# segeschecho/OpenEKFMonoSLAM

Measured on AMD Instinct MI355X. Metric: EKF updates/s (frames/s) at N features, higher is better.
Workload: dtype f32 storage; i8 MFMA with exact i32 sums (downdate) + f64 (B, S, state)

## Files before the change

### openekfmonoslam_amd/csrc/engine.cpp

```cpp
#include "engine.h"
#include "../../include/ekf_test_hooks.h"

#include <cmath>
#include <cstdio>
#include <algorithm>
#include <atomic>
#include <cstdlib>
#include <chrono>
#include <cstring>
#include <mutex>
#include <new>

#include <dlfcn.h>
#include <rccl/rccl.h>

using namespace ekf;

namespace ekf {
void launch_partition(EkfEngine *e, const EkfMatch *src, int M, const uint8_t *flags, EkfMatch *dst1, EkfMatch *dst0,
                      int *cnt1, bool map_update = false, const uint8_t *d_kdesc = nullptr, int *d_idx0 = nullptr,
                      int publish_seq = 0, bool rescue = false);
void launch_outlier_idx(EkfEngine *e, const EkfMatch *src, int M, int *idx);
}

// ... 1374 lines not shown
        }
        (void)hipEventDestroy(e->sw_events[i].first);
        (void)hipEventDestroy(e->sw_events[i].second);
    }
    e->sw_events.clear();
    e->sw_launch.clear();
    e->sw_m.clear();
}

struct StageTimer {
    EkfEngine *e;
    std::vector<hipEvent_t> evs;
    explicit StageTimer(EkfEngine *eng) : e(eng) {}
    ~StageTimer()
    {
        for (auto ev : evs) (void)hipEventDestroy(ev);
    }
    void mark()
    {
        if (!e->timing) return;
        hipEvent_t ev;
        if (hipEventCreate(&ev) != hipSuccess) return;
        (void)hipEventRecord(ev, e->stream);
        evs.push_back(ev);
    }
    void finish()
    {
        if (!e->timing || evs.size() < 7) return;
        (void)hipStreamSynchronize(e->stream);
        double *dst[6] = {&e->times.prediction_ms, &e->times.matching_ms, &e->times.ransac_ms,
                          &e->times.update_li_ms,  &e->times.rescue_ms,   &e->times.update_hi_ms};
        for (int i = 0; i < 6; ++i) {
            float ms = 0.f;
            if (hipEventElapsedTime(&ms, evs[i], evs[i + 1]) == hipSuccess) *dst[i] += ms;
        }
        for (auto ev : evs) (void)hipEventDestroy(ev);
        evs.clear();
        e->times.steps += 1;
        harvest_pu_events(e);
    }
};

static int match_ncc_dev(EkfEngine *e, int *n_matches);

static int detect_step_keypoints(EkfEngine *e);

static int step_dev(EkfEngine *e, const EkfKeypoint *d_kps, const uint8_t *d_desc, int n_kp, EkfStepInfo *info,
                    bool use_ncc = false, bool detect = false)
{
    const bool dev_counts = !use_ncc && !detect && !e->img.valid && !e->keep_step_preds && e->shard_world == 1;
    const bool lean = e->shard_world > 1;
    int *cnt = e->d.counts;
    EkfStepInfo li;
    std::memset(&li, 0, sizeof(li));
    int status = EKF_OK, rc;
    const int retries0 = e->sweep_retries;
    if (!dev_counts && e->err_unread) {
        if ((rc = read_counts(e))) return rc;
        if ((rc = recover_failed_update(e, &status))) return rc;
    }
    bool restarted = false;
restart:
    StageTimer tm(e);
    tm.mark();
    int np = 0;
    if (dev_counts) {
        const bool deferred = launch_predict_with_features(e, e->N);
        launch_hp_rows(e, e->d.plist, e->N, true, cnt + CNT_NPRED, deferred);
    } else {
        launch_predict(e);
        if ((rc = predict_measurements_dev(e, nullptr, e->N, &np, true, lean))) return rc;
    }
    tm.mark();
    int M = 0;
    if (dev_counts) {
        launch_match(e, d_kps, d_desc, e->N, n_kp, cnt + CNT_NPRED, true);
    } else {
        if (detect && (rc = detect_step_keypoints(e))) return rc;
        if (lean) rc = match_sharded_dev(e, use_ncc, d_kps, d_desc, n_kp, &M);
        else rc = use_ncc ? match_ncc_dev(e, &M) : match_dev(e, d_kps, d_desc, n_kp, &M, detect ? cnt + CNT_KP_FOUND : nullptr);
        if (rc) return rc;
    }
    tm.mark();
    if (dev_counts) {
        const int batch = e->cfg.ransac_batch;
        const int seq_r = next_publish_seq(e);
        launch_ransac_batch(e, e->N, 0, batch, cnt + CNT_NMATCH, seq_r);
        if ((rc = wait_counts(e, seq_r))) return rc;
        if (e->h_counts[CNT_ERR] && !restarted) {
            if ((rc = recover_failed_update(e, &status))) return rc;
            restarted = true;
            goto restart;
        }
        np = e->n_pred = e->h_counts[CNT_NPRED];
        M = e->h_counts[CNT_NMATCH];
        for (int h0 = batch, nb = batch * RANSAC_WIDE_FACTOR; !e->h_counts[CNT_RS_DONE] && h0 < M; h0 += nb) {
            launch_ransac_batch(e, M, h0, nb);
            if ((rc = read_counts(e))) return rc;
        }
    } else if (M > 0 && (rc = ransac_dev(e, M, lean))) {
        return rc;
    }
    li.n_predicted = np;
    li.n_matches = M;
    int ni = 0, no = 0;
    if (M > 0) {
        li.n_hypotheses = e->h_counts[CNT_RS_NEXT];
        ni = e->h_counts[CNT_RS_BEST];
        no = M - ni;
        launch_partition(e, e->d.matches, M, e->d.best_flags, e->d.msel, e->d.mout, nullptr, true, d_desc, e->d.work_idx);
    }
    li.n_inliers = ni;
    li.n_outliers = no;
    tm.mark();
    if ((rc = update_dev(e, ni, true, lean))) return rc;
    tm.mark();
    int nr = 0;
    if (no > 0) {
        int nop = 0;
        for (int attempt = 0; attempt < 2; ++attempt) {
            if (dev_counts) {
                launch_predict_features(e, e->d.work_idx, no, false);
                launch_hp_rows(e, e->d.plist_sub, no, false, cnt + CNT_NPRED_SUB);
                const int seq_p = next_publish_seq(e);
                launch_partition(e, e->d.mout, no, e->d.mask, e->d.msel, nullptr, cnt + CNT_NRESC, true, d_desc, nullptr, seq_p, true);
                rc = wait_counts(e, seq_p);
            } else {
                rc = predict_measurements_dev(e, e->d.work_idx, no, &nop, false, lean);
            }
            if (rc) return rc;
            if (!e->h_counts[CNT_ERR]) break;
            if ((rc = recover_failed_update(e, &status))) return rc;
        }
        if (dev_counts) {
            nr = e->h_counts[CNT_NRESC];
        } else if (nop > 0) {
            launch_rescue(e, e->d.mout, no);
            launch_partition(e, e->d.mout, no, e->d.mask, e->d.msel, nullptr, cnt + CNT_NRESC, true, d_desc);
            if ((rc = read_counts(e))) return rc;
            nr = e->h_counts[CNT_NRESC];
        }
    }
    li.n_rescued = nr;
    tm.mark();
    if ((rc = update_dev(e, nr, true, lean))) return rc;
    tm.mark();
    if (dev_counts && e->async_errors) {
        e->err_unread = true;
    } else {
        if ((rc = read_counts(e))) return rc;
        if (detect) {
            e->step_kp_detected = e->h_counts[CNT_KP_FOUND];
            e->step_kp_kept = std::min(e->step_kp_detected, e->kcap);
        }
        if ((rc = recover_failed_update(e, &status))) return rc;
    }
    tm.finish();
    li.status = status;
    li.n_sweep_retries = e->sweep_retries - retries0;
    if (info) *info = li;
    return status;
}

int ekf_set_async_errors(EkfEngine *e, int on)
{
    if (!e) return EKF_ERR_INVALID_ARG;
    e->async_errors = on != 0;
    return EKF_OK;
}

int ekf_set_update_path(EkfEngine *e, int path)
{
    if (!e || path < EKF_UPDATE_PATH_AUTO || path > EKF_UPDATE_PATH_GEMM) return EKF_ERR_INVALID_ARG;
    e->b_path = path;
    return EKF_OK;
}

int ekf_set_sweep_mode(EkfEngine *e, int mode)
{
    if (!e || mode < EKF_SWEEP_PAIRS || mode > EKF_SWEEP_LAUNCHES) return EKF_ERR_INVALID_ARG;
    e->sweep_mode = mode;
    return EKF_OK;
}

int ekf_step(EkfEngine *e, const EkfKeypoint *kps, const uint8_t *desc32, int n_kp, EkfStepInfo *info)
{
    if (!e || n_kp < 0 || (n_kp > 0 && (!kps || !desc32))) return EKF_ERR_INVALID_ARG;
    HIPCHK(hipSetDevice(e->device));
    int rc = upload_keypoints(e, kps, desc32, n_kp);
    if (rc) return rc;
    return step_dev(e, e->d.kps, e->d.kdesc, n_kp, info);
}

// ... 640 lines not shown
```

### openekfmonoslam_amd/csrc/engine.h

```cpp
#pragma once
#include <hip/hip_runtime.h>

#include <atomic>
#include <cstdint>
#include <map>
#include <memory>
#include <mutex>
#include <string>
#include <vector>

#include "../../include/ekf_engine.h"
#include "device_math.h"

namespace ekf {

constexpr int NB = 32;
constexpr int LD_ALIGN = 128;
constexpr int B_SWEEP_MAX = 2048;
constexpr int DX_SPLIT = 16;
constexpr int RANSAC_WIDE_FACTOR = 8;
#ifndef PX_S_VALUE
#define PX_S_VALUE 5
#endif
constexpr int PX_S = PX_S_VALUE;
// ... 241 lines not shown
    ekf::DeviceArrays d;
    ekf::Frames frames;
    ekf::Image img;
    std::string err;
    bool timing = false;
    EkfStageTimes times{};
    hipEvent_t ev[4] = {nullptr, nullptr, nullptr, nullptr};
    std::vector<std::pair<hipEvent_t, hipEvent_t>> pu_events;
    std::vector<double> pu_work;
    std::vector<int> pu_m;
    std::vector<std::pair<int, float>> pu_log;
    std::vector<std::pair<hipEvent_t, hipEvent_t>> sw_events;
    std::vector<int> sw_m;
    std::vector<int> sw_launch;
    double sweep_ms = 0.0, sweep_flops_f64 = 0.0, sweep_flops_b = 0.0;
    long long sweep_panels = 0, sweep_updates = 0, sweep_launches = 0;
    double slice_ms = 0.0;
    std::vector<int> h_counts;
    int *h_mirror = nullptr, *d_mirror = nullptr;
    int mirror_seq = 0;
    std::vector<int> h_type, h_covpos;
};

namespace ekf {

struct XtyArgs {
    const void *X; int ldx; long long xb;
    const void *Y; int ldy; long long yb;
    void *C; int ldc; long long cb;
    void *Ct; int ldct; long long ctb;
    float *Ctf;
    int M, N, K;
    int row0_first, row0_stride, m_lim;
    int tri;
    int tiles_i, tiles_j;
    int tj0;
    int n_split;
    double alpha;
};
void launch_xty(EkfEngine *e, const XtyArgs &a, int batch, bool f32, hipStream_t stream);

#ifdef __HIPCC__
__device__ __forceinline__ bool filter_frozen(const int *counts) { return counts != nullptr && counts[CNT_ERR] != 0; }
#endif

#ifdef __HIPCC__
__device__ __forceinline__ int block_exclusive_scan_1024(int c, int *wtot , int *total)
{
    const int lane = threadIdx.x & 63, wv = threadIdx.x >> 6;
    int x = c;
#pragma unroll
    for (int o = 1; o < 64; o <<= 1) {
        const int y = __shfl_up(x, o, 64);
        if (lane >= o) x += y;
    }
    if (lane == 63) wtot[wv] = x;
    __syncthreads();
    int base = 0, tot = 0;
#pragma unroll
    for (int w = 0; w < 16; ++w) {
        const int t = wtot[w];
        base += w < wv ? t : 0;
        tot += t;
    }
    *total = tot;
    return base + x - c;
}
#endif

void launch_predict(EkfEngine *e);
bool launch_predict_features(EkfEngine *e, const int *d_idx, int count, bool state_only, bool defer_compact = false);
bool launch_predict_with_features(EkfEngine *e, int count);
void launch_hp_rows(EkfEngine *e, const int *d_list, int n_list, bool count_predicted = false, const int *d_count = nullptr, bool from_flags = false);
void launch_match(EkfEngine *e, const EkfKeypoint *kps, const uint8_t *kdesc, int n_pred, int n_kp, const int *d_npred = nullptr,
                  bool with_ransac_init = false, const int *d_nkp = nullptr);
void launch_match_index(EkfEngine *e, int M, const int *d_M = nullptr);
void launch_shard_bounds(EkfEngine *e, const EkfMatch *list, int count);
void launch_shard_bounds_idx(EkfEngine *e, const int *list, const int *d_count);
void launch_match_slots(EkfEngine *e, const EkfKeypoint *kps, const uint8_t *kdesc, int n_kp, int s_lo, int s_hi);
void launch_match_ncc_slots(EkfEngine *e, int s_lo, int s_hi, bool subpix);
void launch_match_compact(EkfEngine *e, const EkfKeypoint *kps, int n_pred);
void launch_match_compact_slots(EkfEngine *e, int n_pred, const EkfKeypoint *d_slot_xy);
void launch_ransac_hyp(EkfEngine *e, int M, int h0, int batch, const int *d_M, int h_lo, int h_hi);
void launch_ransac_select(EkfEngine *e, int M, int h0, int batch, const int *d_M, int publish_seq);
void launch_ransac_batch(EkfEngine *e, int M, int h0, int batch, const int *d_M = nullptr, int publish_seq = 0);
void launch_ransac_init(EkfEngine *e, int M);
void launch_update(EkfEngine *e, int M, bool update_cov);
void launch_p_update_exact(EkfEngine *e, int m, bool use_bc, bool exps_ready = false, bool planes_ready = false);
void launch_round_P_f32(EkfEngine *e);
void launch_diag_extract(EkfEngine *e, float *diag);
void launch_planes_move(EkfEngine *e, bool pack, int m_k, int c_lo, int c_hi, int skip_lo, int skip_hi);
void launch_dx_planes(EkfEngine *e, int m_k);
void launch_slice_columns(EkfEngine *e, int m, int c_lo, int c_hi);
void launch_b_gemm_planes(EkfEngine *e, int m, int c_lo, int c_hi);
void launch_rescue(EkfEngine *e, const EkfMatch *matches, int M);
void launch_state_only_predict(EkfEngine *e, EkfPrediction *d_out);
void launch_add_features(EkfEngine *e, const double *d_uv, int count, double *d_Jpo, double *d_Jhr);
void launch_compact_P(EkfEngine *e, int n_new, const int *d_new2old);
void launch_linearity(EkfEngine *e, double *d_out);
void launch_convert(EkfEngine *e, int fi, int pos, double *d_J, double *d_T3);
void launch_map_points(EkfEngine *e, EkfMapPoint *d_out);
void launch_ncc_pyramid(EkfEngine *e, const uint8_t *d_raw, int stride, int channels);
void launch_ncc_pyramid_on(EkfEngine *e, hipStream_t stream, uint8_t *const px[3], const uint8_t *d_raw, int stride, int channels);
void launch_ncc_capture(EkfEngine *e, const int *d_idx, const double *d_uv, int count);
void launch_ncc_warp_capture(EkfEngine *e, const int *d_idx, const double *d_uv, int count, bool keep);
void launch_match_ncc(EkfEngine *e, int n_pred, bool subpix);
void launch_gate_snapshot(EkfEngine *e, int n_pred);
void launch_detect_cells(EkfEngine *e, int n_gates, int cells_x, int cells_y, long long *d_resp, int *d_xy);
void launch_kp_detect(EkfEngine *e, long long thr, bool masked, unsigned long long *rowmask, EkfKeypoint *out, int cap, int *d_found);
size_t kp_rowmask_words(int w, int h);
void launch_brief(EkfEngine *e, const EkfKeypoint *kps, const int *centres, int n, const int *d_n, uint8_t *desc);
void launch_publish_counts(EkfEngine *e, int *d_mirror, int seq);
__device__ __forceinline__ void publish_counts_block(const int *counts, int *mirror, int seq)
{
    __syncthreads();
    const int t = threadIdx.x;
    if (t < 64) {
        if (t < CNT_COUNT) __hip_atomic_store(&mirror[t], counts[t], __ATOMIC_RELAXED, __HIP_MEMORY_SCOPE_SYSTEM);
        __threadfence_system();
        __builtin_amdgcn_wave_barrier();
        if (t == 0) {
            __threadfence_system();
            __hip_atomic_store(&mirror[CNT_COUNT], seq, __ATOMIC_RELEASE, __HIP_MEMORY_SCOPE_SYSTEM);
        }
    }
}
void launch_pack_predictions(EkfEngine *e, const int *d_list, int n, EkfPrediction *d_out);

}
```

### openekfmonoslam_amd/csrc/kernels_match.hip

```cpp
#include "engine.h"
#include "gate.h"

namespace ekf {

__global__ void __launch_bounds__(256)
k_match(const int *plist, const double *uv_tab, const double *S_tab, const uint8_t *feat_desc,
        const EkfKeypoint *kps, const uint8_t *kdesc, int n_kp, double coef, int *mt_valid, int *mt_kp,
        float *mt_dist, int desc_bytes, int desc_f32, const int *d_npred, int slot0, const int *d_nkp)
{
    if (d_npred && slot0 + (int)blockIdx.x >= *d_npred) return;
    if (d_nkp) n_kp = min(*d_nkp, n_kp);
    __shared__ Gate g;
    __shared__ uint32_t qd[1024];
    constexpr int PASS = 8;
    __shared__ int c_idx[256 * PASS];
    __shared__ double c_dist[256 * PASS];
    __shared__ int wave_cnt[PASS][4];
    __shared__ int s_list_n, s_front;
    __shared__ float s_dfront, s_dback;
    __shared__ double s_min;

    const int k = slot0 + (int)blockIdx.x, tid = threadIdx.x;
    const int fi = plist[k];
    if (tid == 0) {
        float axes[2];
        double angle;
        ellipse_from_cov(S_tab + 4 * fi, axes, &angle);
        const int aw = (int)rintf(axes[0]), ah = (int)rintf(axes[1]);
        gate_from_ellipse((float)uv_tab[2 * fi], (float)uv_tab[2 * fi + 1], aw, ah, angle, &g);
        s_list_n = 0; s_front = -1; s_dfront = 0.f; s_dback = 0.f; s_min = -1.0;
    }
    const int words = desc_bytes / 4;
    for (int w = tid; w < words; w += 256) qd[w] = ((const uint32_t *)(feat_desc + (size_t)fi * desc_bytes))[w];
    const int lane = tid & 63, wv = tid >> 6;
    for (int base = 0; base < n_kp; base += 256 * PASS) {
        float kx[PASS], ky[PASS];
#pragma unroll
        for (int i = 0; i < PASS; ++i) {
            const int j = min(base + i * 256 + tid, n_kp - 1);
            kx[i] = kps[j].x;
            ky[i] = kps[j].y;
        }
        __syncthreads();
        bool inside[PASS];
        double dist[PASS];
        int rank[PASS];
#pragma unroll
        for (int i = 0; i < PASS; ++i) {
            const int j = base + i * 256 + tid;
            const double px = (double)kx[i], py = (double)ky[i];
            const double a1x = px - g.f1x, a1y = py - g.f1y, a2x = px - g.f2x, a2y = py - g.f2y;
            const double ns = sqrt(a1x * a1x + a1y * a1y) + sqrt(a2x * a2x + a2y * a2y);
            inside[i] = j < n_kp && ns <= g.two_major;
            dist[i] = 0.0;
            if (inside[i]) {
                const uint32_t *cd = (const uint32_t *)(kdesc + (size_t)j * desc_bytes);
                if (desc_f32) {
                    double acc = 0.0;
                    for (int w = 0; w < words; ++w) {
                        const float subs = __uint_as_float(qd[w]) - __uint_as_float(cd[w]);
                        acc += (double)(subs * subs);
                    }
                    dist[i] = sqrt(acc);
                } else {
                    int d = 0;
                    for (int w = 0; w < words; ++w) d += __popc(cd[w] ^ qd[w]);
                    dist[i] = (double)d;
                }
            }
            const unsigned long long bal = __ballot(inside[i]);
            rank[i] = __popcll(bal & ((1ull << lane) - 1ull));
            if (lane == 0) wave_cnt[i][wv] = __popcll(bal);
        }
        __syncthreads();
        int nc = 0;
#pragma unroll
        for (int i = 0; i < PASS; ++i) {
#pragma unroll
            for (int w = 0; w < 4; ++w) {
                const int c = wave_cnt[i][w];
                if (w == wv && inside[i]) {
                    c_idx[nc + rank[i]] = base + i * 256 + tid;
                    c_dist[nc + rank[i]] = dist[i];
                }
// ... 76 lines not shown
        return;
    }
    k_match<<<n_pred, 256, 0, e->stream>>>(e->d.plist, e->d.pred_uv, e->d.pred_S, e->d.feat_desc, kps,
                                           kdesc, n_kp, e->cfg.par.matchingCompCoefSecondBestVSFirst,
                                           e->d.mt_valid, e->d.mt_kp, e->d.mt_dist, e->desc_bytes, e->desc_f32 ? 1 : 0, d_npred, 0,
                                           d_nkp);
    k_match_compact<<<1, 1024, 0, e->stream>>>(e->d.plist, n_pred, e->d.mt_valid, e->d.mt_kp, e->d.mt_dist,
                                               kps, 0, e->d.matches, e->d.counts + CNT_NMATCH, d_npred,
                                               with_ransac_init ? e->d.counts : nullptr, e->d.match_of_feat, e->d.best_flags, e->N);
}

void launch_match_slots(EkfEngine *e, const EkfKeypoint *kps, const uint8_t *kdesc, int n_kp, int s_lo, int s_hi)
{
    if (s_hi <= s_lo) return;
    k_match<<<s_hi - s_lo, 256, 0, e->stream>>>(e->d.plist, e->d.pred_uv, e->d.pred_S, e->d.feat_desc, kps, kdesc, n_kp,
                                                e->cfg.par.matchingCompCoefSecondBestVSFirst, e->d.mt_valid, e->d.mt_kp, e->d.mt_dist,
                                                e->desc_bytes, e->desc_f32 ? 1 : 0, nullptr, s_lo, nullptr);
}

void launch_match_compact(EkfEngine *e, const EkfKeypoint *kps, int n_pred)
{
    if (n_pred <= 0) {
        (void)hipMemsetAsync(e->d.counts + CNT_NMATCH, 0, sizeof(int), e->stream);
        return;
    }
    k_match_compact<<<1, 1024, 0, e->stream>>>(e->d.plist, n_pred, e->d.mt_valid, e->d.mt_kp, e->d.mt_dist, kps, 0, e->d.matches,
                                               e->d.counts + CNT_NMATCH, nullptr, nullptr, nullptr, nullptr, 0);
}

void launch_match_compact_slots(EkfEngine *e, int n_pred, const EkfKeypoint *d_slot_xy)
{
    k_match_compact<<<1, 1024, 0, e->stream>>>(e->d.plist, n_pred, e->d.mt_valid, e->d.mt_kp, e->d.mt_dist, d_slot_xy,
                                               1, e->d.matches, e->d.counts + CNT_NMATCH, nullptr, nullptr, nullptr, nullptr, 0);
}

__global__ void __launch_bounds__(256) k_match_index(const EkfMatch *m, int M, int *match_of_feat, int N, const int *d_M)
{
    if (d_M) M = *d_M;
    const int i = blockIdx.x * 256 + threadIdx.x;
    if (i >= M) return;
    const int f = m[i].featureIndex;
    if (f >= 0 && f < N) atomicMin(&match_of_feat[f], i);
}

__global__ void __launch_bounds__(256) k_fill_int(int *p, int n, int v)
{
    const int i = blockIdx.x * 256 + threadIdx.x;
    if (i < n) p[i] = v;
}

void launch_match_index(EkfEngine *e, int M, const int *d_M)
{
    if (e->N <= 0) return;
    if (M > 0) k_match_index<<<(M + 255) / 256, 256, 0, e->stream>>>(e->d.matches, M, e->d.match_of_feat, e->N, d_M);
}

__global__ void __launch_bounds__(1024)
k_partition(const EkfMatch *src, int M, const uint8_t *flags, EkfMatch *dst1, EkfMatch *dst0, int *cnt1, const uint8_t *kdesc,
            uint8_t *feat_desc, unsigned *times_matched, int desc_bytes, int *idx0, const int *counts, int *mirror,
            int publish_seq, uint8_t *rescue_mask, const int *vis, const double *uv_tab, const double *S_tab, double chi2)
{
    __shared__ int wtot[16];
    const int tid = threadIdx.x;
    if (filter_frozen(counts)) {
        if (publish_seq > 0) publish_counts_block(counts, mirror, publish_seq);
        return;
    }
    const int per = (M + 1023) / 1024;
    const int b = tid * per, e = min(M, b + per);
    if (rescue_mask) {
        for (int i = b; i < e; ++i) {
            const int fi = src[i].featureIndex;
            const double d0 = src[i].imagePos[0] - uv_tab[2 * fi];
            const double d1 = src[i].imagePos[1] - uv_tab[2 * fi + 1];
            double Si[4];
            inv2(S_tab + 4 * fi, Si);
            const double t0 = d0 * Si[0] + d1 * Si[2];
            const double t1 = d0 * Si[1] + d1 * Si[3];
            const double v = t0 * d0 + t1 * d1;
            rescue_mask[i] = (vis[fi] && v < chi2) ? 1 : 0;
        }
        flags = rescue_mask;
    }
    int c = 0;
    for (int i = b; i < e; ++i) c += flags[i] ? 1 : 0;
    int total;
    int p1 = block_exclusive_scan_1024(c, wtot, &total);
    int p0 = b - p1;
    for (int i = b; i < e; ++i) {
        if (flags[i]) dst1[p1++] = src[i];
        else if (dst0) {
            if (idx0) idx0[p0] = src[i].featureIndex;
            dst0[p0++] = src[i];
        }
    }
    if (tid == 1023 && cnt1) *cnt1 = total;
    if (publish_seq > 0) publish_counts_block(counts, mirror, publish_seq);
    if (!times_matched) return;
    __syncthreads();
    const int count = total;
    for (int i = tid; i < count; i += 1024) {
        const int fi = dst1[i].featureIndex, kp = dst1[i].keypointIndex;
        atomicAdd(&times_matched[fi], 1u);
        if (kp >= 0 && kdesc) {
            const uint32_t *sd = (const uint32_t *)(kdesc + (size_t)kp * desc_bytes);
            uint32_t *dd = (uint32_t *)(feat_desc + (size_t)fi * desc_bytes);
            for (int w = 0; w < desc_bytes / 4; ++w) dd[w] = sd[w];
        }
    }
}

void launch_partition(EkfEngine *e, const EkfMatch *src, int M, const uint8_t *flags, EkfMatch *dst1, EkfMatch *dst0,
                      int *cnt1, bool map_update, const uint8_t *d_kdesc, int *d_idx0, int publish_seq, bool rescue)
{
    if (M <= 0) {
        if (cnt1) (void)hipMemsetAsync(cnt1, 0, sizeof(int), e->stream);
        return;
    }
    k_partition<<<1, 1024, 0, e->stream>>>(src, M, flags, dst1, dst0, cnt1, d_kdesc, e->d.feat_desc,
                                           map_update ? e->d.feat_times_matched : nullptr, e->desc_bytes, d_idx0, e->d.counts,
                                           e->d_mirror, e->d_mirror ? publish_seq : 0, rescue ? e->d.mask : nullptr, e->d.pred_vis,
                                           e->d.pred_uv, e->d.pred_S, e->cfg.par.ransacChi2Threshold);
}





__global__ void k_shard_bounds(const EkfMatch *list, int count, const int *feat_begin, int world, int *counts)
{
    const int r = threadIdx.x;
    const int f = r <= world ? feat_begin[r] : 0;
    int lo = 0, hi = r <= world ? count : 0;
    while (lo < hi) {
        const int mid = (lo + hi) >> 1;
        if (list[mid].featureIndex < f) lo = mid + 1;
        else hi = mid;
    }
    if (r <= world) counts[CNT_SHARD0 + r] = lo;
    __shared__ int bad;
    if (threadIdx.x == 0) bad = 0;
    __syncthreads();
    for (int i = threadIdx.x; i + 1 < count; i += blockDim.x)
        if (list[i].featureIndex >= list[i + 1].featureIndex) bad = 1;
    __syncthreads();
    if (bad && r == world) counts[CNT_SHARD0 + r] = -1;
}

__global__ void k_shard_bounds_idx(const int *list, const int *d_count, const int *feat_begin, int world, int *counts)
{
    const int r = threadIdx.x, count = *d_count;
    const int f = r <= world ? feat_begin[r] : 0;
    int lo = 0, hi = r <= world ? count : 0;
    while (lo < hi) {
        const int mid = (lo + hi) >> 1;
        if (list[mid] < f) lo = mid + 1;
        else hi = mid;
    }
    if (r <= world) counts[CNT_SHARD0 + r] = lo;
}

void launch_shard_bounds_idx(EkfEngine *e, const int *list, const int *d_count)
{
    k_shard_bounds_idx<<<1, 64, 0, e->stream>>>(list, d_count, e->d.shard_feat, e->shard_world, e->d.counts);
}

void launch_shard_bounds(EkfEngine *e, const EkfMatch *list, int count)
{
    k_shard_bounds<<<1, 64, 0, e->stream>>>(list, count, e->d.shard_feat, e->shard_world, e->d.counts);
}

__global__ void __launch_bounds__(256) k_outlier_idx(const EkfMatch *src, int M, int *idx)
{
    const int i = blockIdx.x * 256 + threadIdx.x;
    if (i < M) idx[i] = src[i].featureIndex;
}

void launch_outlier_idx(EkfEngine *e, const EkfMatch *src, int M, int *idx)
{
    if (M > 0) k_outlier_idx<<<(M + 255) / 256, 256, 0, e->stream>>>(src, M, idx);
}

__global__ void k_publish_counts(const int *counts, int *mirror, int seq)
{
    const int t = threadIdx.x;
    if (t < CNT_COUNT) __hip_atomic_store(&mirror[t], counts[t], __ATOMIC_RELAXED, __HIP_MEMORY_SCOPE_SYSTEM);
    __threadfence_system();
    __builtin_amdgcn_wave_barrier();
    if (t == 0) {
        __threadfence_system();
        __hip_atomic_store(&mirror[CNT_COUNT], seq, __ATOMIC_RELEASE, __HIP_MEMORY_SCOPE_SYSTEM);
    }
// ... 9 lines not shown
```

### openekfmonoslam_amd/csrc/kernels_predict.hip

```cpp
#include "engine.h"

namespace ekf {

__device__ void predict_prepare_serial(double *st, double *sG);

__global__ void __launch_bounds__(256) k_predict_prepare(double *st, ParD par, const int *counts)
{
    __shared__ double sG[13 * 6];
    if (filter_frozen(counts)) return;
    const double dt = 1.0;
    const double ln = par.linearAccelSD * par.linearAccelSD * dt * dt;
    const double an = par.angularAccelSD * par.angularAccelSD * dt * dt;
    if (blockIdx.x != 0) return;
    if (threadIdx.x == 0) predict_prepare_serial(st, sG);
    __syncthreads();
    if (threadIdx.x < 169) {
        const int i = threadIdx.x / 13, j = threadIdx.x % 13;
        double s = 0.0;
        for (int k = 0; k < 6; ++k) s += (sG[i * 6 + k] * (k < 3 ? ln : an)) * sG[j * 6 + k];
        st[ST_GQG + i * 13 + j] = s;
    }
}

__device__ void predict_prepare_serial(double *st, double *sG)
{
    const double dt = 1.0;
    double *x = st + ST_X;
    double *F = st + ST_F, *GQG = st + ST_GQG;
    for (int i = 0; i < 169; ++i) F[i] = 0.0;
    for (int i = 0; i < 13; ++i) F[i * 13 + i] = 1.0;
    for (int i = 0; i < 3; ++i) F[i * 13 + i + 7] = dt;
    double w[3] = {x[10] * dt, x[11] * dt, x[12] * dt};
    double nw = sqrt(w[0] * w[0] + w[1] * w[1] + w[2] * w[2]);
    double qr[4];
    if (nw < EKF_EPSILON) {
        qr[0] = 1; qr[1] = 0; qr[2] = 0; qr[3] = 0;
    } else {
        const double s = sin(nw / 2);
        qr[0] = cos(nw / 2); qr[1] = s * w[0] / nw; qr[2] = s * w[1] / nw; qr[3] = s * w[2] / nw;
    }
    {
        const double qw = qr[0], qx = qr[1], qy = qr[2], qz = qr[3];
        const double Fq[16] = {qw, -qx, -qy, -qz, qx, qw, qz, -qy, qy, -qz, qw, qx, qz, qy, -qx, qw};
        for (int i = 0; i < 4; ++i)
            for (int j = 0; j < 4; ++j) F[(3 + i) * 13 + 3 + j] = Fq[i * 4 + j];
    }
    double G[13 * 6];
    for (int i = 0; i < 78; ++i) G[i] = 0.0;
    if (fabs(x[10]) < EKF_EPSILON && fabs(x[11]) < EKF_EPSILON && fabs(x[12]) < EKF_EPSILON) {
        for (int i = 0; i < 3; ++i) F[(i + 10) * 13 + i + 10] = 0.0;
    } else {
        const double om = sqrt(x[10] * x[10] + x[11] * x[11] + x[12] * x[12]);
        const double *q = x + 3;
        const double Qm[16] = {q[0], -q[1], -q[2], -q[3], q[1], q[0], -q[3], q[2],
                               q[2], q[3], q[0], -q[1], q[3], -q[2], q[1], q[0]};
        const double sh = sin(om * dt / 2.0), ch = cos(om * dt / 2.0);
        double D[12];
        for (int a = 0; a < 3; ++a) {
            const double wa = x[10 + a];
            D[a] = (-dt / 2.0) * (wa / om) * sh;
            for (int b = 0; b < 3; ++b) {
                const double wb = x[10 + b];
                double v;
                if (a == b)
                    v = (dt / 2.0) * wa * wa / (om * om) * ch + (1.0 / om) * (1.0 - wa * wa / (om * om)) * sh;
                else
                    v = (wa * wb / (om * om)) * ((dt / 2.0) * ch - (1.0 / om) * sh);
                D[3 + a * 3 + b] = v;
            }
        }
        for (int i = 0; i < 4; ++i)
            for (int j = 0; j < 3; ++j) {
                double s = 0.0;
                for (int k = 0; k < 4; ++k) s += Qm[i * 4 + k] * D[k * 3 + j];
                F[(3 + i) * 13 + 10 + j] = s;
                G[(3 + i) * 6 + 3 + j] = s;
            }
    }
    for (int i = 0; i < 3; ++i) {
        G[(i + 7) * 6 + i] = 1.0;
        G[(i + 10) * 6 + i + 3] = 1.0;
        G[i * 6 + i] = 1.0 * dt;
    }
    for (int i = 0; i < 78; ++i) sG[i] = G[i];
    (void)GQG;
    for (int i = 0; i < 3; ++i) x[i] += x[7 + i] * dt;
    {
        const double q1w = x[3], q1x = x[4], q1y = x[5], q1z = x[6];
        const double q2w = qr[0], q2x = qr[1], q2y = qr[2], q2z = qr[3];
        x[3] = q1w * q2w - q1x * q2x - q1y * q2y - q1z * q2z;
        x[4] = q1w * q2x + q1x * q2w + q1y * q2z - q1z * q2y;
        x[5] = q1w * q2y - q1x * q2z + q1y * q2w + q1z * q2x;
        x[6] = q1w * q2z + q1x * q2y - q1y * q2x + q1z * q2w;
    }
    quat_to_rot(x + 3, st + ST_R);
}

template <typename T>
__device__ __forceinline__ void predict_cov_body(const int bx, T *P, int ld, int n, const double *st, RowMap rm)
{
    __shared__ double sF[169];
    __shared__ double sC[169];
    __shared__ double sFP[169];
    const int tid = threadIdx.x;
    for (int i = tid; i < 169; i += 256) sF[i] = st[ST_F + i];
    if (bx == 0) {
        for (int i = tid; i < 169; i += 256) sC[i] = (double)P[(size_t)(i / 13) * ld + (i % 13)];
        __syncthreads();
        if (tid < 169) {
            const int i = tid / 13, j = tid % 13;
            double s = 0.0;
            for (int k = 0; k < 13; ++k) s += sF[i * 13 + k] * sC[k * 13 + j];
            sFP[tid] = s;
        }
        __syncthreads();
        if (tid < 169) {
            const int i = tid / 13, j = tid % 13;
            if (i <= j) {
                double s = 0.0;
                for (int k = 0; k < 13; ++k) s += sFP[i * 13 + k] * sF[j * 13 + k];
                const T v = (T)(s + st[ST_GQG + tid]);
                P[(size_t)i * ld + j] = v;
                P[(size_t)j * ld + i] = v;
            }
        }
        return;
    }
    __syncthreads();
    const int j = 13 + (bx - 1) * 256 + tid;
    if (j >= n) return;
    const bool mine = owns_row(rm, j);
    T *prow = P + (size_t)local_row(rm, j) * ld;
    double col[13], row[13];
#pragma unroll
    for (int a = 0; a < 13; ++a) col[a] = (double)P[(size_t)a * ld + j];
#pragma unroll
    for (int a = 0; a < 13; ++a) row[a] = mine ? (double)prow[a] : 0.0;
#pragma unroll
    for (int a = 0; a < 13; ++a) {
        double s = 0.0, t = 0.0;
#pragma unroll
        for (int b = 0; b < 13; ++b) {
            s += sF[a * 13 + b] * col[b];
            t += row[b] * sF[a * 13 + b];
        }
        P[(size_t)a * ld + j] = (T)s;
        if (mine) prow[a] = (T)t;
    }
}

template <typename T>
__global__ void __launch_bounds__(256) k_predict_cov(T *P, int ld, int n, const double *st, RowMap rm)
{
    predict_cov_body<T>((int)blockIdx.x, P, ld, n, st, rm);
}

void launch_predict(EkfEngine *e)
{
    k_predict_prepare<<<1, 256, 0, e->stream>>>(e->d.state, e->par, nullptr);
    const int nb = 1 + (e->n > 13 ? (e->n - 13 + 255) / 256 : 0);
    if (e->f32)
        k_predict_cov<float><<<nb, 256, 0, e->stream>>>((float *)e->d.P, e->ldP, e->n, e->d.state, e->rm);
    else
        k_predict_cov<double><<<nb, 256, 0, e->stream>>>((double *)e->d.P, e->ldP, e->n, e->d.state, e->rm);
}

template <int BLOCK>
__device__ __forceinline__ void
predict_features_body(const int bx, const double *st, const CamD &cam, const double *feat_pos, const int *feat_type, const int *idx,
                      int count, int *flag, int *vis, double *uv_tab, double *Hs_tab, double *Hf_tab, int *vis_full, int *list, int *out_count)
{
    __shared__ int wtot[16];
    const int w = bx * BLOCK + threadIdx.x;
    if (list && threadIdx.x < 16) wtot[threadIdx.x] = 0;
    bool ok = false;
    int fi = 0;
    if (w < count) {
        fi = idx ? idx[w] : w;
// ... 304 lines not shown
```

### openekfmonoslam_amd/csrc/kernels_ransac.hip

```cpp
#include "engine.h"

namespace ekf {

constexpr int HYP_THREADS = 512;

template <typename T>
__global__ void __launch_bounds__(HYP_THREADS)
k_ransac_hyp(const double *st, CamD cam, double thr, const double *feat_pos, const int *feat_type,
             const int *feat_covpos, int N, const T *HP, int ld, const double *uv_tab, const double *S_tab,
             const EkfMatch *matches, int M, const int *match_of_feat, int h0, int *hyp_count, uint8_t *hyp_flags,
             int mcap, const int *d_M, int h_lo, int h_hi)
{
    __shared__ double sx[13], sRt[9], sRinv[9], sw[2];
    __shared__ int s_cnt[HYP_THREADS / 64];
    if (d_M) M = *d_M;
    const int h = h0 + blockIdx.x;
    if (h >= M) return;
    if (h < h_lo || h >= h_hi) return;
    const int tid = threadIdx.x;
    const int fi = matches[h].featureIndex;
    const T *g0 = HP + (size_t)(2 * fi) * ld;
    const T *g1 = g0 + ld;
    if (tid == 0) {
        double S[4] = {S_tab[4 * fi] - 1.0 + cam.pixelErrorX, S_tab[4 * fi + 1], S_tab[4 * fi + 2],
                       S_tab[4 * fi + 3] - 1.0 + cam.pixelErrorX};
        double Si[4];
        inv2(S, Si);
        const double ax = matches[h].imagePos[0] - uv_tab[2 * fi];
        const double ay = matches[h].imagePos[1] - uv_tab[2 * fi + 1];
        const double n0 = fabs(ax) > EKF_DELTA ? ax : 0.0;
        const double n1 = fabs(ay) > EKF_DELTA ? ay : 0.0;
        const double w0 = Si[0] * n0 + Si[1] * n1;
        const double w1 = Si[2] * n0 + Si[3] * n1;
        sw[0] = w0;
        sw[1] = w1;
        double x[13];
        for (int i = 0; i < 13; ++i) {
            const double dx = (double)g0[i] * w0 + (double)g1[i] * w1;
            x[i] = st[ST_X + i] + (fabs(dx) > EKF_DELTA ? dx : 0.0);
            sx[i] = x[i];
        }
        double R[9];
        quat_to_rot(x + 3, R);
        for (int i = 0; i < 3; ++i)
            for (int j = 0; j < 3; ++j) sRt[j * 3 + i] = R[i * 3 + j];
        inv3(R, sRinv);
    }
    __syncthreads();
    const double w0 = sw[0], w1 = sw[1];
    uint8_t *flags = hyp_flags + (size_t)blockIdx.x * mcap;
    const int nthr = blockDim.x;
    for (int k = tid; k < M; k += nthr) flags[k] = 0;
    __syncthreads();
    int cnt = 0;
    for (int f = tid; f < N; f += nthr) {
        const int mi = match_of_feat[f];
        if (mi >= M) continue;
        const int type = feat_type[f], pos = feat_covpos[f], d = feat_dim(type);
        double fp[6];
        for (int a = 0; a < 6; ++a) fp[a] = feat_pos[6 * f + a];
        for (int a = 0; a < d; ++a) {
            const double dx = (double)g0[pos + a] * w0 + (double)g1[pos + a] * w1;
            if (fabs(dx) > EKF_DELTA) fp[a] += dx;
        }
        double uv[2];
        int ok = 0;
        if (predict_pixel(cam, sx, sRt, sRinv, fp, type, uv)) {
            const double xd = matches[mi].imagePos[0] - uv[0];
            const double yd = matches[mi].imagePos[1] - uv[1];
            ok = sqrt(xd * xd + yd * yd) < thr ? 1 : 0;
        }
        flags[mi] = (uint8_t)ok;
        cnt += ok;
    }
    cnt = wave_sum_i(cnt);
    if ((tid & 63) == 0) s_cnt[tid >> 6] = cnt;
    __syncthreads();
    if (tid == 0) {
        int tot = 0;
        for (int w = 0; w < nthr / 64; ++w) tot += s_cnt[w];
        hyp_count[blockIdx.x] = tot;
    }
}

__global__ void __launch_bounds__(256)
k_ransac_select(int *counts, const int *hyp_count, const uint8_t *hyp_flags, uint8_t *best_flags, int M, int h0,
                int batch, int mcap, double prob, const int *d_M, int *mirror, int publish_seq)
{
    if (d_M) M = *d_M;
    const int tid = threadIdx.x;
    int best = counts[CNT_RS_BEST], besth = counts[CNT_RS_BESTH], nhyp = counts[CNT_RS_NHYP], next = counts[CNT_RS_NEXT];
    __syncthreads();
    int last = -1;
    bool stop = false, done = false;
    for (int b = 0; b < batch; ++b) {
        const int i = h0 + b;
        if (!((unsigned)i < (unsigned)nhyp && i < M)) {
            stop = true;
            done = true;
            break;
        }
        const int ns = hyp_count[b];
        if (ns > best) {
            best = ns;
            besth = i;
            const double e = 1.0 - (double)ns / (double)M;
            nhyp = (int)(log(1.0 - prob) / log(1.0 - (1.0 - e)));
            last = b;
        }
        next = i + 1;
    }
    if (!stop) {
        const int i = h0 + batch;
        if (!((unsigned)i < (unsigned)nhyp && i < M)) done = true;
    }
    if (last >= 0)
        for (int k = tid; k < M; k += 256) best_flags[k] = hyp_flags[(size_t)last * mcap + k];
    if (tid == 0) {
        counts[CNT_RS_BEST] = best;
        counts[CNT_RS_BESTH] = besth;
        counts[CNT_RS_NHYP] = nhyp;
        counts[CNT_RS_NEXT] = next;
        if (done) counts[CNT_RS_DONE] = 1;
    }
    if (publish_seq > 0) publish_counts_block(counts, mirror, publish_seq);
}

__global__ void __launch_bounds__(256) k_ransac_init(int *counts, int *match_of_feat, uint8_t *best_flags, int N, int M)
{
    const int i = blockIdx.x * 256 + threadIdx.x;
    if (i == 0) {
        counts[CNT_RS_BEST] = 0;
        counts[CNT_RS_BESTH] = -1;
        counts[CNT_RS_NHYP] = 1000;
        counts[CNT_RS_NEXT] = 0;
        counts[CNT_RS_DONE] = 0;
    }
    if (i < N) match_of_feat[i] = 0x7fffffff;
    if (i < M) best_flags[i] = 0;
}

void launch_ransac_init(EkfEngine *e, int M)
{
    const int n = max(max(e->N, M), 1);
    k_ransac_init<<<(n + 255) / 256, 256, 0, e->stream>>>(e->d.counts, e->d.match_of_feat, e->d.best_flags, e->N, M);
}

void launch_ransac_hyp(EkfEngine *e, int M, int h0, int batch, const int *d_M, int h_lo, int h_hi)
{
    const int nb = batch;
    const double thr = e->cfg.par.ransacThresholdPredictDistance;
    if (e->f32 && !e->exact)
        k_ransac_hyp<float><<<nb, e->N > 256 ? HYP_THREADS : 256, 0, e->stream>>>(e->d.state, e->cam, thr, e->d.feat_pos, e->d.feat_type,
                                                       e->d.feat_covpos, e->N, (const float *)e->d.HP, e->ldP,
                                                       e->d.pred_uv, e->d.pred_S, e->d.matches, M,
                                                       e->d.match_of_feat, h0, e->d.hyp_count, e->d.hyp_flags,
                                                       e->mcap, d_M, h_lo, h_hi);
    else
        k_ransac_hyp<double><<<nb, e->N > 256 ? HYP_THREADS : 256, 0, e->stream>>>(e->d.state, e->cam, thr, e->d.feat_pos, e->d.feat_type,
                                                        e->d.feat_covpos, e->N, (const double *)e->d.HP, e->ldP,
                                                        e->d.pred_uv, e->d.pred_S, e->d.matches, M,
                                                        e->d.match_of_feat, h0, e->d.hyp_count, e->d.hyp_flags,
                                                        e->mcap, d_M, h_lo, h_hi);
}

void launch_ransac_select(EkfEngine *e, int M, int h0, int batch, const int *d_M, int publish_seq)
{
    k_ransac_select<<<1, 256, 0, e->stream>>>(e->d.counts, e->d.hyp_count, e->d.hyp_flags, e->d.best_flags, M, h0,
                                              batch, e->mcap, e->cfg.par.ransacAllInliersProbability, d_M, e->d_mirror,
                                              e->d_mirror ? publish_seq : 0);
}

void launch_ransac_batch(EkfEngine *e, int M, int h0, int batch, const int *d_M, int publish_seq)
{
    launch_ransac_hyp(e, M, h0, batch, d_M, 0, 0x7fffffff);
    launch_ransac_select(e, M, h0, batch, d_M, publish_seq);
}

__global__ void __launch_bounds__(256)
k_rescue(const EkfMatch *m, int M, const int *vis, const double *uv_tab, const double *S_tab, double chi2,
         uint8_t *mask)
{
    const int i = blockIdx.x * 256 + threadIdx.x;
    if (i >= M) return;
    const int fi = m[i].featureIndex;
    const double d0 = m[i].imagePos[0] - uv_tab[2 * fi];
    const double d1 = m[i].imagePos[1] - uv_tab[2 * fi + 1];
    double Si[4];
    inv2(S_tab + 4 * fi, Si);
    const double t0 = d0 * Si[0] + d1 * Si[2];
    const double t1 = d0 * Si[1] + d1 * Si[3];
    const double v = t0 * d0 + t1 * d1;
    mask[i] = (vis[fi] && v < chi2) ? 1 : 0;
}

void launch_rescue(EkfEngine *e, const EkfMatch *matches, int M)
{
    if (M <= 0) return;
    k_rescue<<<(M + 255) / 256, 256, 0, e->stream>>>(matches, M, e->d.pred_vis, e->d.pred_uv, e->d.pred_S,
                                                     e->cfg.par.ransacChi2Threshold, e->d.mask);
}

}
```

Baseline: 1203.

## Fuse match partition into RANSAC select kernel and parallelize predict prepare

When the first RANSAC batch already finishes, the select kernel now runs with 1024 threads and partitions matches into inlier/outlier lists itself, including the map descriptor and times-matched update. The host then skips the separate partition launch. The predict-prepare kernel also splits its serial F/G build and its state/rotation update across two threads, with shared staging, instead of one thread doing all of it. This trades a larger select block and more shared-memory staging for one fewer launch on the frame path and a shorter serial section.

```diff
diff --git a/openekfmonoslam_amd/csrc/engine.cpp b/openekfmonoslam_amd/csrc/engine.cpp
--- a/openekfmonoslam_amd/csrc/engine.cpp
+++ b/openekfmonoslam_amd/csrc/engine.cpp
@@ -1480,10 +1480,11 @@
         if (rc) return rc;
     }
     tm.mark();
+    bool partitioned = false;
     if (dev_counts) {
         const int batch = e->cfg.ransac_batch;
         const int seq_r = next_publish_seq(e);
-        launch_ransac_batch(e, e->N, 0, batch, cnt + CNT_NMATCH, seq_r);
+        launch_ransac_batch(e, e->N, 0, batch, cnt + CNT_NMATCH, seq_r, true, d_desc);
         if ((rc = wait_counts(e, seq_r))) return rc;
         if (e->h_counts[CNT_ERR] && !restarted) {
             if ((rc = recover_failed_update(e, &status))) return rc;
@@ -1492,6 +1493,7 @@
         }
         np = e->n_pred = e->h_counts[CNT_NPRED];
         M = e->h_counts[CNT_NMATCH];
+        partitioned = e->h_counts[CNT_RS_DONE] != 0;
         for (int h0 = batch, nb = batch * RANSAC_WIDE_FACTOR; !e->h_counts[CNT_RS_DONE] && h0 < M; h0 += nb) {
             launch_ransac_batch(e, M, h0, nb);
             if ((rc = read_counts(e))) return rc;
@@ -1506,7 +1508,7 @@
         li.n_hypotheses = e->h_counts[CNT_RS_NEXT];
         ni = e->h_counts[CNT_RS_BEST];
         no = M - ni;
-        launch_partition(e, e->d.matches, M, e->d.best_flags, e->d.msel, e->d.mout, nullptr, true, d_desc, e->d.work_idx);
+        if (!partitioned) launch_partition(e, e->d.matches, M, e->d.best_flags, e->d.msel, e->d.mout, nullptr, true, d_desc, e->d.work_idx);
     }
     li.n_inliers = ni;
     li.n_outliers = no;
diff --git a/openekfmonoslam_amd/csrc/engine.h b/openekfmonoslam_amd/csrc/engine.h
--- a/openekfmonoslam_amd/csrc/engine.h
+++ b/openekfmonoslam_amd/csrc/engine.h
@@ -347,8 +347,10 @@
 void launch_match_compact(EkfEngine *e, const EkfKeypoint *kps, int n_pred);
 void launch_match_compact_slots(EkfEngine *e, int n_pred, const EkfKeypoint *d_slot_xy);
 void launch_ransac_hyp(EkfEngine *e, int M, int h0, int batch, const int *d_M, int h_lo, int h_hi);
-void launch_ransac_select(EkfEngine *e, int M, int h0, int batch, const int *d_M, int publish_seq);
-void launch_ransac_batch(EkfEngine *e, int M, int h0, int batch, const int *d_M = nullptr, int publish_seq = 0);
+void launch_ransac_select(EkfEngine *e, int M, int h0, int batch, const int *d_M, int publish_seq, bool partition = false,
+                          const uint8_t *d_kdesc = nullptr);
+void launch_ransac_batch(EkfEngine *e, int M, int h0, int batch, const int *d_M = nullptr, int publish_seq = 0, bool partition = false,
+                         const uint8_t *d_kdesc = nullptr);
 void launch_ransac_init(EkfEngine *e, int M);
 void launch_update(EkfEngine *e, int M, bool update_cov);
 void launch_p_update_exact(EkfEngine *e, int m, bool use_bc, bool exps_ready = false, bool planes_ready = false);
diff --git a/openekfmonoslam_amd/csrc/kernels_match.hip b/openekfmonoslam_amd/csrc/kernels_match.hip
--- a/openekfmonoslam_amd/csrc/kernels_match.hip
+++ b/openekfmonoslam_amd/csrc/kernels_match.hip
@@ -1,5 +1,6 @@
 #include "engine.h"
 #include "gate.h"
+#include "partition.h"
 
 namespace ekf {
 
@@ -242,32 +243,10 @@
         }
         flags = rescue_mask;
     }
-    int c = 0;
-    for (int i = b; i < e; ++i) c += flags[i] ? 1 : 0;
-    int total;
-    int p1 = block_exclusive_scan_1024(c, wtot, &total);
-    int p0 = b - p1;
-    for (int i = b; i < e; ++i) {
-        if (flags[i]) dst1[p1++] = src[i];
-        else if (dst0) {
-            if (idx0) idx0[p0] = src[i].featureIndex;
-            dst0[p0++] = src[i];
-        }
-    }
+    const int total = partition_matches(src, M, flags, dst1, dst0, idx0, wtot);
     if (tid == 1023 && cnt1) *cnt1 = total;
     if (publish_seq > 0) publish_counts_block(counts, mirror, publish_seq);
-    if (!times_matched) return;
-    __syncthreads();
-    const int count = total;
-    for (int i = tid; i < count; i += 1024) {
-        const int fi = dst1[i].featureIndex, kp = dst1[i].keypointIndex;
-        atomicAdd(&times_matched[fi], 1u);
-        if (kp >= 0 && kdesc) {
-            const uint32_t *sd = (const uint32_t *)(kdesc + (size_t)kp * desc_bytes);
-            uint32_t *dd = (uint32_t *)(feat_desc + (size_t)fi * desc_bytes);
-            for (int w = 0; w < desc_bytes / 4; ++w) dd[w] = sd[w];
-        }
-    }
+    if (times_matched) map_update_matched(dst1, total, kdesc, feat_desc, times_matched, desc_bytes);
 }
 
 void launch_partition(EkfEngine *e, const EkfMatch *src, int M, const uint8_t *flags, EkfMatch *dst1, EkfMatch *dst0,
diff --git a/openekfmonoslam_amd/csrc/kernels_predict.hip b/openekfmonoslam_amd/csrc/kernels_predict.hip
--- a/openekfmonoslam_amd/csrc/kernels_predict.hip
+++ b/openekfmonoslam_amd/csrc/kernels_predict.hip
@@ -2,51 +2,31 @@
 
 namespace ekf {
 
-__device__ void predict_prepare_serial(double *st, double *sG);
-
-__global__ void __launch_bounds__(256) k_predict_prepare(double *st, ParD par, const int *counts)
-{
-    __shared__ double sG[13 * 6];
-    if (filter_frozen(counts)) return;
+__device__ __forceinline__ void quat_of_rotation(const double *x, double *qr)
+{
     const double dt = 1.0;
-    const double ln = par.linearAccelSD * par.linearAccelSD * dt * dt;
-    const double an = par.angularAccelSD * par.angularAccelSD * dt * dt;
-    if (blockIdx.x != 0) return;
-    if (threadIdx.x == 0) predict_prepare_serial(st, sG);
-    __syncthreads();
-    if (threadIdx.x < 169) {
-        const int i = threadIdx.x / 13, j = threadIdx.x % 13;
-        double s = 0.0;
-        for (int k = 0; k < 6; ++k) s += (sG[i * 6 + k] * (k < 3 ? ln : an)) * sG[j * 6 + k];
-        st[ST_GQG + i * 13 + j] = s;
-    }
-}
-
-__device__ void predict_prepare_serial(double *st, double *sG)
-{
-    const double dt = 1.0;
-    double *x = st + ST_X;
-    double *F = st + ST_F, *GQG = st + ST_GQG;
-    for (int i = 0; i < 169; ++i) F[i] = 0.0;
-    for (int i = 0; i < 13; ++i) F[i * 13 + i] = 1.0;
-    for (int i = 0; i < 3; ++i) F[i * 13 + i + 7] = dt;
     double w[3] = {x[10] * dt, x[11] * dt, x[12] * dt};
     double nw = sqrt(w[0] * w[0] + w[1] * w[1] + w[2] * w[2]);
-    double qr[4];
     if (nw < EKF_EPSILON) {
         qr[0] = 1; qr[1] = 0; qr[2] = 0; qr[3] = 0;
     } else {
         const double s = sin(nw / 2);
         qr[0] = cos(nw / 2); qr[1] = s * w[0] / nw; qr[2] = s * w[1] / nw; qr[3] = s * w[2] / nw;
     }
+}
+
+__device__ void predict_prepare_FG(const double *x, double *F, double *G)
+{
+    const double dt = 1.0;
+    for (int i = 0; i < 3; ++i) F[i * 13 + i + 7] = dt;
+    double qr[4];
+    quat_of_rotation(x, qr);
     {
         const double qw = qr[0], qx = qr[1], qy = qr[2], qz = qr[3];
         const double Fq[16] = {qw, -qx, -qy, -qz, qx, qw, qz, -qy, qy, -qz, qw, qx, qz, qy, -qx, qw};
         for (int i = 0; i < 4; ++i)
             for (int j = 0; j < 4; ++j) F[(3 + i) * 13 + 3 + j] = Fq[i * 4 + j];
     }
-    double G[13 * 6];
-    for (int i = 0; i < 78; ++i) G[i] = 0.0;
     if (fabs(x[10]) < EKF_EPSILON && fabs(x[11]) < EKF_EPSILON && fabs(x[12]) < EKF_EPSILON) {
         for (int i = 0; i < 3; ++i) F[(i + 10) * 13 + i + 10] = 0.0;
     } else {
@@ -82,18 +62,54 @@
         G[(i + 10) * 6 + i + 3] = 1.0;
         G[i * 6 + i] = 1.0 * dt;
     }
-    for (int i = 0; i < 78; ++i) sG[i] = G[i];
-    (void)GQG;
-    for (int i = 0; i < 3; ++i) x[i] += x[7 + i] * dt;
+}
+
+__device__ void predict_prepare_state(const double *x, double *xn, double *R)
+{
+    const double dt = 1.0;
+    double qr[4];
+    quat_of_rotation(x, qr);
+    for (int i = 0; i < 3; ++i) xn[i] = x[i] + x[7 + i] * dt;
     {
         const double q1w = x[3], q1x = x[4], q1y = x[5], q1z = x[6];
         const double q2w = qr[0], q2x = qr[1], q2y = qr[2], q2z = qr[3];
-        x[3] = q1w * q2w - q1x * q2x - q1y * q2y - q1z * q2z;
-        x[4] = q1w * q2x + q1x * q2w + q1y * q2z - q1z * q2y;
-        x[5] = q1w * q2y - q1x * q2z + q1y * q2w + q1z * q2x;
-        x[6] = q1w * q2z + q1x * q2y - q1y * q2x + q1z * q2w;
-    }
-    quat_to_rot(x + 3, st + ST_R);
+        xn[3] = q1w * q2w - q1x * q2x - q1y * q2y - q1z * q2z;
+        xn[4] = q1w * q2x + q1x * q2w + q1y * q2z - q1z * q2y;
+        xn[5] = q1w * q2y - q1x * q2z + q1y * q2w + q1z * q2x;
+        xn[6] = q1w * q2z + q1x * q2y - q1y * q2x + q1z * q2w;
+    }
+    quat_to_rot(xn + 3, R);
+}
+
+__global__ void __launch_bounds__(256) k_predict_prepare(double *st, ParD par, const int *counts)
+{
+    __shared__ double sG[13 * 6], sF[169], sX[7], sR[9];
+    if (filter_frozen(counts)) return;
+    const double dt = 1.0;
+    const double ln = par.linearAccelSD * par.linearAccelSD * dt * dt;
+    const double an = par.angularAccelSD * par.angularAccelSD * dt * dt;
+    if (blockIdx.x != 0) return;
+    const int tid = threadIdx.x;
+    double x[13];
+    if (tid == 0 || tid == 64)
+        for (int i = 0; i < 13; ++i) x[i] = st[ST_X + i];
+    if (tid < 169) sF[tid] = tid / 13 == tid % 13 ? 1.0 : 0.0;
+    if (tid < 78) sG[tid] = 0.0;
+    __syncthreads();
+    if (tid == 0) predict_prepare_FG(x, sF, sG);
+    else if (tid == 64) predict_prepare_state(x, sX, sR);
+    __syncthreads();
+    if (tid < 169) {
+        const int i = tid / 13, j = tid % 13;
+        double s = 0.0;
+        for (int k = 0; k < 6; ++k) s += (sG[i * 6 + k] * (k < 3 ? ln : an)) * sG[j * 6 + k];
+        st[ST_GQG + i * 13 + j] = s;
+        st[ST_F + tid] = sF[tid];
+    } else if (tid < 176) {
+        st[ST_X + tid - 169] = sX[tid - 169];
+    } else if (tid < 185) {
+        st[ST_R + tid - 176] = sR[tid - 176];
+    }
 }
 
 template <typename T>
diff --git a/openekfmonoslam_amd/csrc/kernels_ransac.hip b/openekfmonoslam_amd/csrc/kernels_ransac.hip
--- a/openekfmonoslam_amd/csrc/kernels_ransac.hip
+++ b/openekfmonoslam_amd/csrc/kernels_ransac.hip
@@ -1,4 +1,5 @@
 #include "engine.h"
+#include "partition.h"
 
 namespace ekf {
 
@@ -83,13 +84,26 @@
     }
 }
 
-__global__ void __launch_bounds__(256)
+struct SelectPartition {
+    const EkfMatch *src;
+    EkfMatch *dst1, *dst0;
+    int *idx0;
+    const uint8_t *kdesc;
+    uint8_t *feat_desc;
+    unsigned *times_matched;
+    int desc_bytes;
+};
+
+__global__ void __launch_bounds__(1024)
 k_ransac_select(int *counts, const int *hyp_count, const uint8_t *hyp_flags, uint8_t *best_flags, int M, int h0,
-                int batch, int mcap, double prob, const int *d_M, int *mirror, int publish_seq)
-{
+                int batch, int mcap, double prob, const int *d_M, int *mirror, int publish_seq, SelectPartition part)
+{
+    __shared__ int wtot[16];
     if (d_M) M = *d_M;
-    const int tid = threadIdx.x;
+    const int tid = threadIdx.x, nthr = blockDim.x;
+    if (tid < 16) wtot[tid] = 0;
     int best = counts[CNT_RS_BEST], besth = counts[CNT_RS_BESTH], nhyp = counts[CNT_RS_NHYP], next = counts[CNT_RS_NEXT];
+    const bool frozen = part.src != nullptr && filter_frozen(counts);
     __syncthreads();
     int last = -1;
     bool stop = false, done = false;
@@ -115,7 +129,7 @@
         if (!((unsigned)i < (unsigned)nhyp && i < M)) done = true;
     }
     if (last >= 0)
-        for (int k = tid; k < M; k += 256) best_flags[k] = hyp_flags[(size_t)last * mcap + k];
+        for (int k = tid; k < M; k += nthr) best_flags[k] = hyp_flags[(size_t)last * mcap + k];
     if (tid == 0) {
         counts[CNT_RS_BEST] = best;
         counts[CNT_RS_BESTH] = besth;
@@ -124,6 +138,10 @@
         if (done) counts[CNT_RS_DONE] = 1;
     }
     if (publish_seq > 0) publish_counts_block(counts, mirror, publish_seq);
+    if (part.src == nullptr || !done || frozen || M <= 0) return;
+    __syncthreads();
+    const int total = partition_matches(part.src, M, best_flags, part.dst1, part.dst0, part.idx0, wtot);
+    map_update_matched(part.dst1, total, part.kdesc, part.feat_desc, part.times_matched, part.desc_bytes);
 }
 
 __global__ void __launch_bounds__(256) k_ransac_init(int *counts, int *match_of_feat, uint8_t *best_flags, int N, int M)
@@ -164,17 +182,21 @@
                                                         e->mcap, d_M, h_lo, h_hi);
 }
 
-void launch_ransac_select(EkfEngine *e, int M, int h0, int batch, const int *d_M, int publish_seq)
-{
-    k_ransac_select<<<1, 256, 0, e->stream>>>(e->d.counts, e->d.hyp_count, e->d.hyp_flags, e->d.best_flags, M, h0,
-                                              batch, e->mcap, e->cfg.par.ransacAllInliersProbability, d_M, e->d_mirror,
-                                              e->d_mirror ? publish_seq : 0);
-}
-
-void launch_ransac_batch(EkfEngine *e, int M, int h0, int batch, const int *d_M, int publish_seq)
+void launch_ransac_select(EkfEngine *e, int M, int h0, int batch, const int *d_M, int publish_seq, bool partition, const uint8_t *d_kdesc)
+{
+    SelectPartition part = {};
+    if (partition)
+        part = SelectPartition{e->d.matches, e->d.msel, e->d.mout, e->d.work_idx, d_kdesc, e->d.feat_desc, e->d.feat_times_matched,
+                               e->desc_bytes};
+    k_ransac_select<<<1, partition ? 1024 : 256, 0, e->stream>>>(e->d.counts, e->d.hyp_count, e->d.hyp_flags, e->d.best_flags, M, h0,
+                                                                 batch, e->mcap, e->cfg.par.ransacAllInliersProbability, d_M, e->d_mirror,
+                                                                 e->d_mirror ? publish_seq : 0, part);
+}
+
+void launch_ransac_batch(EkfEngine *e, int M, int h0, int batch, const int *d_M, int publish_seq, bool partition, const uint8_t *d_kdesc)
 {
     launch_ransac_hyp(e, M, h0, batch, d_M, 0, 0x7fffffff);
-    launch_ransac_select(e, M, h0, batch, d_M, publish_seq);
+    launch_ransac_select(e, M, h0, batch, d_M, publish_seq, partition, d_kdesc);
 }
 
 __global__ void __launch_bounds__(256)
diff --git a/openekfmonoslam_amd/csrc/partition.h b/openekfmonoslam_amd/csrc/partition.h
--- /dev/null
+++ b/openekfmonoslam_amd/csrc/partition.h
@@ -0,0 +1,42 @@
+#pragma once
+#include "engine.h"
+
+namespace ekf {
+
+__device__ __forceinline__ int partition_matches(const EkfMatch *src, int M, const uint8_t *flags, EkfMatch *dst1, EkfMatch *dst0, int *idx0,
+                                                 int *wtot)
+{
+    const int nthr = blockDim.x, tid = threadIdx.x;
+    const int per = (M + nthr - 1) / nthr;
+    const int b = min(M, tid * per), e = min(M, b + per);
+    int c = 0;
+    for (int i = b; i < e; ++i) c += flags[i] ? 1 : 0;
+    int total;
+    int p1 = block_exclusive_scan_1024(c, wtot, &total);
+    int p0 = b - p1;
+    for (int i = b; i < e; ++i) {
+        if (flags[i]) dst1[p1++] = src[i];
+        else if (dst0) {
+            if (idx0) idx0[p0] = src[i].featureIndex;
+            dst0[p0++] = src[i];
+        }
+    }
+    return total;
+}
+
+__device__ __forceinline__ void map_update_matched(const EkfMatch *sel, int count, const uint8_t *kdesc, uint8_t *feat_desc,
+                                                   unsigned *times_matched, int desc_bytes)
+{
+    __syncthreads();
+    for (int i = threadIdx.x; i < count; i += blockDim.x) {
+        const int fi = sel[i].featureIndex, kp = sel[i].keypointIndex;
+        atomicAdd(&times_matched[fi], 1u);
+        if (kp >= 0 && kdesc) {
+            const uint32_t *sd = (const uint32_t *)(kdesc + (size_t)kp * desc_bytes);
+            uint32_t *dd = (uint32_t *)(feat_desc + (size_t)fi * desc_bytes);
+            for (int w = 0; w < desc_bytes / 4; ++w) dd[w] = sd[w];
+        }
+    }
+}
+
+}
```

Result: no change. 1211, median of 6 (+0.7%).
